# XIAOCHIZI/spark-bam

Measured on AMD Instinct MI355X. Metric: decompressed GB/s + records/sec (inflate+boundary check) at 1/2/4/8 MI355X, higher is better.
Workload: dtype u8

## Files before the change

### spark-bam_amd/csrc/inflate.hip

```cpp
#include "sbh_internal.h"

namespace sbh {
namespace {

#ifndef SBH_HUFF_WAVES
#define SBH_HUFF_WAVES 4
#endif
constexpr int LIT_FAST = 10;
constexpr int DIST_FAST = 8;
constexpr int CL_FAST = 7;
constexpr int PDIST_FAST = 10;
constexpr int WAVES = SBH_HUFF_WAVES;
#ifndef SBH_LZ_THREADS
#define SBH_LZ_THREADS 512
#endif
constexpr uint32_t LZ_THREADS = SBH_LZ_THREADS;
#ifndef SBH_LZ_SHORT
#define SBH_LZ_SHORT 32
#endif
constexpr uint32_t LZ_SHORT = SBH_LZ_SHORT;
static_assert(LZ_SHORT <= 33, "k_lz finds a short match's start within 32 slots back");
constexpr uint32_t TOK_PAIR = 1u << 24;
constexpr uint32_t TOK_MATCH = 0x80000000u;

// ... 1136 lines not shown

#ifndef SBH_ASM_REDO
#define SBH_ASM_REDO 1
#endif
__device__ __forceinline__ LaneRun redo_asm(const WaveSmem &t, const uint32_t *stage, uint32_t A, uint32_t stop,
                                            uint32_t limit, const Ckpt &ck, const LaneRun &sp) {
  const uint32_t stop2 = stop < limit ? stop : limit;
  if (A >= stop2) return LaneRun{A >= limit ? LR_PAST : LR_RUN, A, 0, 0};
  const uint32_t tabb = uni((uint32_t)reinterpret_cast<uintptr_t>(t.tab));
  const uint32_t stb = uni((uint32_t)reinterpret_cast<uintptr_t>(stage) + 8u);
  const uint32_t pkb = uni((uint32_t)reinterpret_cast<uintptr_t>(&t.pk[0][11]));
  const uint32_t sentb = uni((uint32_t)reinterpret_cast<uintptr_t>(t.sent));
  const uint32_t sentd = sentb + 288u * 4u;
  uint32_t pos = A, lo = stage[A >> 5], hi = stage[(A >> 5) + 1];
  uint32_t vt = 0, tselb = tabb, ntok = 0, acc = 0;
  const uint32_t bad_e = 1u | PE_SPECIAL;
  const uint32_t k1 = ck.p1, k2 = ck.p2, k3 = ck.p3;
  uint32_t e = 0, bits, a, nx, x, ex, val, np, tmp, r15, q, p11, p12, p13, p14, p15, d, sh;
  uint64_t sA, sB, sC, sD, sE, sv;
  asm volatile(
      "s_mov_b64 %[sv], exec\n"
      "L_top%=:\n\t"
      "v_alignbit_b32 %[bits], %[hi], %[lo], %[pos]\n\t"
      "v_and_b32 %[a], 0x3ff, %[bits]\n\t"
      "v_lshl_add_u32 %[a], %[a], 2, %[tselb]\n\t"
      "ds_read_b32 %[e], %[a]\n\t"
      "v_lshrrev_b32 %[a], 5, %[pos]\n\t"
      "v_lshl_add_u32 %[a], %[a], 2, %[stb]\n\t"
      "ds_read_b32 %[nx], %[a]\n\t"
      "v_cmp_eq_u32 %[sA], 0, %[vt]\n\t"
      "v_cmp_ge_u32 %[sC], %[pos], %[stop]\n\t"
      "v_cmp_eq_u32 %[sB], %[pos], %[k1]\n\t"
      "v_cmp_eq_u32 %[sE], %[pos], %[k2]\n\t"
      "s_or_b64 %[sC], %[sC], %[sB]\n\t"
      "v_cmp_eq_u32 %[sB], %[pos], %[k3]\n\t"
      "s_or_b64 %[sC], %[sC], %[sE]\n\t"
      "s_or_b64 %[sC], %[sC], %[sB]\n\t"
      "s_and_b64 %[sC], %[sC], %[sA]\n"
      "L_nock%=:\n\t"
      "s_waitcnt lgkmcnt(1)\n\t"
      "v_cmp_gt_i32 %[sD], 0, %[e]\n\t"
      "s_and_b64 %[sD], %[sD], exec\n\t"
      "s_cbranch_scc0 L_nosp%=\n\t"
      "v_and_b32 %[tmp], 0x4000, %[e]\n\t"
      "v_cmp_ne_u32 %[sB], 0, %[tmp]\n\t"
      "s_and_b64 %[sB], %[sB], %[sD]\n\t"
      "s_cbranch_scc0 L_nosp%=\n\t"
      "s_and_saveexec_b64 %[sB], %[sB]\n\t"
      "v_bfrev_b32 %[r15], %[bits]\n\t"
      "v_lshrrev_b32 %[r15], 17, %[r15]\n\t"
      "v_lshrrev_b32 %[q], 6, %[vt]\n\t"
      "v_add_u32 %[q], %[pkb], %[q]\n\t"
      "ds_read_b32 %[p11], %[q]\n\t"
      "ds_read_b32 %[p12], %[q] offset:4\n\t"
      "ds_read_b32 %[p13], %[q] offset:8\n\t"
      "ds_read_b32 %[p14], %[q] offset:12\n\t"
      "ds_read_b32 %[p15], %[q] offset:16\n\t"
      "s_waitcnt lgkmcnt(0)\n\t"
      "v_mov_b32 %[d], %[p11]\n\t"
      "v_mov_b32 %[sh], 4\n\t"
      "v_lshrrev_b32 %[tmp], 16, %[p11]\n\t"
      "v_cmp_le_u32 vcc, %[tmp], %[r15]\n\t"
      "s_nop 1\n\t"
      "v_cndmask_b32_e32 %[d], %[d], %[p12], vcc\n\t"
      "v_cndmask_b32_e64 %[sh], %[sh], 3, vcc\n\t"
      "v_lshrrev_b32 %[tmp], 16, %[p12]\n\t"
      "v_cmp_le_u32 vcc, %[tmp], %[r15]\n\t"
      "s_nop 1\n\t"
      "v_cndmask_b32_e32 %[d], %[d], %[p13], vcc\n\t"
      "v_cndmask_b32_e64 %[sh], %[sh], 2, vcc\n\t"
      "v_lshrrev_b32 %[tmp], 16, %[p13]\n\t"
      "v_cmp_le_u32 vcc, %[tmp], %[r15]\n\t"
      "s_nop 1\n\t"
      "v_cndmask_b32_e32 %[d], %[d], %[p14], vcc\n\t"
      "v_cndmask_b32_e64 %[sh], %[sh], 1, vcc\n\t"
      "v_lshrrev_b32 %[tmp], 16, %[p14]\n\t"
      "v_cmp_le_u32 vcc, %[tmp], %[r15]\n\t"
      "s_nop 1\n\t"
      "v_cndmask_b32_e32 %[d], %[d], %[p15], vcc\n\t"
      "v_cndmask_b32_e64 %[sh], %[sh], 0, vcc\n\t"
      "v_lshrrev_b32 %[tmp], %[sh], %[r15]\n\t"
      "v_add_u32 %[tmp], %[tmp], %[d]\n\t"
      "v_and_b32 %[tmp], 0xffff, %[tmp]\n\t"
      "v_min_u32 %[tmp], 0x13f, %[tmp]\n\t"
      "v_cmp_ne_u32 vcc, 0, %[vt]\n\t"
      "v_mov_b32 %[q], %[sentd]\n\t"
      "v_mov_b32 %[d], %[sentb]\n\t"
      "v_cndmask_b32_e32 %[q], %[d], %[q], vcc\n\t"
      "v_lshl_add_u32 %[tmp], %[tmp], 2, %[q]\n\t"
      "ds_read_b32 %[e], %[tmp]\n\t"
      "v_lshrrev_b32 %[tmp], 16, %[p15]\n\t"
      "v_cmp_ge_u32 vcc, %[r15], %[tmp]\n\t"
      "s_waitcnt lgkmcnt(0)\n\t"
      "s_nop 1\n\t"
      "v_cndmask_b32_e32 %[e], %[e], %[bad_e], vcc\n\t"
      "s_mov_b64 exec, %[sB]\n\t"
      "v_cmp_gt_i32 %[sD], 0, %[e]\n"
      "L_nosp%=:\n\t"
      "s_or_b64 %[sD], %[sD], %[sC]\n\t"
      "s_andn2_b64 exec, exec, %[sD]\n\t"
      "s_cbranch_execz L_end%=\n\t"
      "v_and_b32 %[tmp], 31, %[e]\n\t"
      "v_bfe_u32 %[x], %[e], 5, 4\n\t"
      "v_bfe_u32 %[ex], %[bits], %[e], %[x]\n\t"
      "v_add3_u32 %[np], %[pos], %[tmp], %[x]\n\t"
      "v_add_u32_sdwa %[val], %[ex], %[e] dst_sel:DWORD dst_unused:UNUSED_PAD src0_sel:DWORD src1_sel:WORD_1\n\t"
      "v_xor_b32 %[tmp], %[np], %[pos]\n\t"
      "v_cmp_lt_u32 vcc, 31, %[tmp]\n\t"
      "v_and_b32 %[vt], 0x1000, %[e]\n\t"
      "v_mov_b32 %[pos], %[np]\n\t"
      "s_waitcnt lgkmcnt(0)\n\t"
      "v_cndmask_b32_e32 %[lo], %[lo], %[hi], vcc\n\t"
      "v_cndmask_b32_e32 %[hi], %[hi], %[nx], vcc\n\t"
      "v_addc_co_u32_e64 %[ntok], vcc, 0, %[ntok], %[sA]\n\t"
      "v_add_u32 %[tselb], %[tabb], %[vt]\n\t"
      "v_mad_u32_u24 %[acc], %[vt], %[val], %[acc]\n\t"
      "v_and_b32 %[tmp], 0x400, %[e]\n\t"
      "v_lshl_add_u32 %[acc], %[tmp], 2, %[acc]\n\t"
      "s_branch L_top%=\n"
      "L_end%=:\n\t"
      "s_waitcnt lgkmcnt(0)\n\t"
      "s_mov_b64 exec, %[sv]"
      : [pos] "+v"(pos), [lo] "+v"(lo), [hi] "+v"(hi), [vt] "+v"(vt), [tselb] "+v"(tselb), [ntok] "+v"(ntok),
        [acc] "+v"(acc), [e] "+v"(e), [bits] "=&v"(bits), [a] "=&v"(a), [nx] "=&v"(nx), [x] "=&v"(x),
        [ex] "=&v"(ex), [val] "=&v"(val), [np] "=&v"(np), [tmp] "=&v"(tmp), [r15] "=&v"(r15), [q] "=&v"(q),
        [p11] "=&v"(p11), [p12] "=&v"(p12), [p13] "=&v"(p13), [p14] "=&v"(p14), [p15] "=&v"(p15), [d] "=&v"(d),
        [sh] "=&v"(sh), [sA] "=&s"(sA), [sB] "=&s"(sB), [sC] "=&s"(sC), [sD] "=&s"(sD), [sE] "=&s"(sE),
        [sv] "=&s"(sv)
      : [stop] "v"(stop2), [k1] "v"(k1), [k2] "v"(k2), [k3] "v"(k3), [tabb] "s"(tabb), [stb] "s"(stb),
        [pkb] "s"(pkb), [sentb] "s"(sentb), [sentd] "s"(sentd), [bad_e] "v"(bad_e)
      : "vcc", "scc", "memory");
  LaneRun r{LR_RUN, pos, ntok, ntok + (acc >> 12)};
  if (vt == 0 && (pos >= stop2 || pos == k1 || pos == k2 || pos == k3)) {
    if (pos < stop2) {
      const bool one = pos == k1;
      const bool two = pos == k2;
      r.ntok += sp.ntok - (one ? CK1 : two ? CK2 : CK3);
      r.nout += sp.nout - ck_out(ck, one, two);
      r.st = sp.st;
      r.exit = sp.exit;
    } else if (pos >= limit) {
      r.st = LR_PAST;
    }
  } else {
    r.st = (vt == 0 && (e & PE_EOB)) ? LR_EOB : LR_DEAD;
    r.exit = pos + (e & 31);
  }
  return r;
}

#ifndef SBH_ASM_EMIT
#define SBH_ASM_EMIT 1
#endif
__device__ __forceinline__ void emit_asm(const WaveSmem &t, const uint32_t *stage, uint32_t A, uint32_t stop,
                                         uint32_t limit, uint32_t *tk, uint32_t tidx, uint32_t out0, uint32_t &bad) {
  const uint32_t stop2 = stop < limit ? stop : limit;
  if (A >= stop2) return;
  const uint32_t tabb = uni((uint32_t)reinterpret_cast<uintptr_t>(t.tab));
  const uint32_t stb = uni((uint32_t)reinterpret_cast<uintptr_t>(stage) + 8u);
  const uint32_t pkb = uni((uint32_t)reinterpret_cast<uintptr_t>(&t.pk[0][11]));
  const uint32_t sentb = uni((uint32_t)reinterpret_cast<uintptr_t>(t.sent));
  const uint32_t sentd = sentb + 288u * 4u;
  const uint64_t tkp = reinterpret_cast<uint64_t>(tk);
  const uint64_t tkb = (uint64_t)uni((uint32_t)tkp) | (uint64_t)uni((uint32_t)(tkp >> 32)) << 32;
  uint32_t pos = A, lo = stage[A >> 5], hi = stage[(A >> 5) + 1];
  uint32_t vt = 0, tselb = tabb, ntok = 0, acc = 0, ml = 0, voff = tidx * 4u, badv = 0, cnt = 0;
  const uint32_t om1 = out0 - 1u;
  const uint32_t bad_e = 1u | PE_SPECIAL;
  uint32_t e = 0, bits, a, nx, x, ex, val, np, tmp, r15, q, p11, p12, p13, p14, p15, d, sh, vtok, vb;
  uint64_t sA, sB, sC, sD, sE, sL, sBad, sv;
  asm volatile(
      "s_mov_b64 %[sv], exec\n\t"
      "s_mov_b64 %[sBad], 0\n"
      "L_top%=:\n\t"
      "v_alignbit_b32 %[bits], %[hi], %[lo], %[pos]\n\t"
      "v_and_b32 %[a], 0x3ff, %[bits]\n\t"
      "v_lshl_add_u32 %[a], %[a], 2, %[tselb]\n\t"
      "ds_read_b32 %[e], %[a]\n\t"
      "v_lshrrev_b32 %[a], 5, %[pos]\n\t"
      "v_lshl_add_u32 %[a], %[a], 2, %[stb]\n\t"
      "ds_read_b32 %[nx], %[a]\n\t"
      "v_cmp_eq_u32 %[sA], 0, %[vt]\n\t"
      "v_cmp_ge_u32 %[sC], %[pos], %[stop]\n\t"
      "s_and_b64 %[sC], %[sC], %[sA]\n"
      "L_nock%=:\n\t"
      "s_waitcnt lgkmcnt(1)\n\t"
      "v_cmp_gt_i32 %[sD], 0, %[e]\n\t"
      "s_and_b64 %[sD], %[sD], exec\n\t"
      "s_cbranch_scc0 L_nosp%=\n\t"
      "v_and_b32 %[tmp], 0x4000, %[e]\n\t"
      "v_cmp_ne_u32 %[sB], 0, %[tmp]\n\t"
      "s_and_b64 %[sB], %[sB], %[sD]\n\t"
      "s_cbranch_scc0 L_nosp%=\n\t"
      "s_and_saveexec_b64 %[sB], %[sB]\n\t"
      "v_bfrev_b32 %[r15], %[bits]\n\t"
      "v_lshrrev_b32 %[r15], 17, %[r15]\n\t"
      "v_lshrrev_b32 %[q], 6, %[vt]\n\t"
      "v_add_u32 %[q], %[pkb], %[q]\n\t"
      "ds_read_b32 %[p11], %[q]\n\t"
      "ds_read_b32 %[p12], %[q] offset:4\n\t"
      "ds_read_b32 %[p13], %[q] offset:8\n\t"
      "ds_read_b32 %[p14], %[q] offset:12\n\t"
      "ds_read_b32 %[p15], %[q] offset:16\n\t"
      "s_waitcnt lgkmcnt(0)\n\t"
      "v_mov_b32 %[d], %[p11]\n\t"
      "v_mov_b32 %[sh], 4\n\t"
      "v_lshrrev_b32 %[tmp], 16, %[p11]\n\t"
      "v_cmp_le_u32 vcc, %[tmp], %[r15]\n\t"
      "s_nop 1\n\t"
      "v_cndmask_b32_e32 %[d], %[d], %[p12], vcc\n\t"
      "v_cndmask_b32_e64 %[sh], %[sh], 3, vcc\n\t"
      "v_lshrrev_b32 %[tmp], 16, %[p12]\n\t"
      "v_cmp_le_u32 vcc, %[tmp], %[r15]\n\t"
      "s_nop 1\n\t"
      "v_cndmask_b32_e32 %[d], %[d], %[p13], vcc\n\t"
      "v_cndmask_b32_e64 %[sh], %[sh], 2, vcc\n\t"
      "v_lshrrev_b32 %[tmp], 16, %[p13]\n\t"
      "v_cmp_le_u32 vcc, %[tmp], %[r15]\n\t"
      "s_nop 1\n\t"
      "v_cndmask_b32_e32 %[d], %[d], %[p14], vcc\n\t"
      "v_cndmask_b32_e64 %[sh], %[sh], 1, vcc\n\t"
      "v_lshrrev_b32 %[tmp], 16, %[p14]\n\t"
      "v_cmp_le_u32 vcc, %[tmp], %[r15]\n\t"
      "s_nop 1\n\t"
      "v_cndmask_b32_e32 %[d], %[d], %[p15], vcc\n\t"
      "v_cndmask_b32_e64 %[sh], %[sh], 0, vcc\n\t"
      "v_lshrrev_b32 %[tmp], %[sh], %[r15]\n\t"
      "v_add_u32 %[tmp], %[tmp], %[d]\n\t"
      "v_and_b32 %[tmp], 0xffff, %[tmp]\n\t"
      "v_min_u32 %[tmp], 0x13f, %[tmp]\n\t"
      "v_cmp_ne_u32 vcc, 0, %[vt]\n\t"
      "v_mov_b32 %[q], %[sentd]\n\t"
      "v_mov_b32 %[d], %[sentb]\n\t"
      "v_cndmask_b32_e32 %[q], %[d], %[q], vcc\n\t"
      "v_lshl_add_u32 %[tmp], %[tmp], 2, %[q]\n\t"
      "ds_read_b32 %[e], %[tmp]\n\t"
      "v_lshrrev_b32 %[tmp], 16, %[p15]\n\t"
      "v_cmp_ge_u32 vcc, %[r15], %[tmp]\n\t"
      "s_waitcnt lgkmcnt(0)\n\t"
      "s_nop 1\n\t"
      "v_cndmask_b32_e32 %[e], %[e], %[bad_e], vcc\n\t"
      "s_mov_b64 exec, %[sB]\n\t"
      "v_cmp_gt_i32 %[sD], 0, %[e]\n"
      "L_nosp%=:\n\t"
      "s_or_b64 %[sD], %[sD], %[sC]\n\t"
      "s_andn2_b64 exec, exec, %[sD]\n\t"
      "s_cbranch_execz L_end%=\n\t"
      "v_and_b32 %[tmp], 31, %[e]\n\t"
      "v_bfe_u32 %[x], %[e], 5, 4\n\t"
      "v_bfe_u32 %[ex], %[bits], %[e], %[x]\n\t"
      "v_add3_u32 %[np], %[pos], %[tmp], %[x]\n\t"
      "v_add_u32_sdwa %[val], %[ex], %[e] dst_sel:DWORD dst_unused:UNUSED_PAD src0_sel:DWORD src1_sel:WORD_1\n\t"
      "v_and_b32 %[vt], 0x1000, %[e]\n\t"
      "v_xor_b32 %[tmp], %[np], %[pos]\n\t"
      "v_cmp_ne_u32 %[sL], 0, %[vt]\n\t"
      "v_cmp_lt_u32 vcc, 31, %[tmp]\n\t"
      "v_mov_b32 %[pos], %[np]\n\t"
      "v_lshlrev_b32 %[vtok], 8, %[val]\n\t"
      "v_and_b32 %[tmp], 0x600, %[e]\n\t"
      "v_lshl_or_b32 %[vtok], %[tmp], 14, %[vtok]\n\t"
      "v_or_b32 %[np], %[ml], %[val]\n\t"
      "v_lshl_add_u32 %[ml], %[val], 16, %[mlk]\n\t"
      "v_cndmask_b32_e64 %[vtok], %[np], %[vtok], %[sA]\n\t"
      "s_waitcnt lgkmcnt(0)\n\t"
      "v_cndmask_b32_e32 %[lo], %[lo], %[hi], vcc\n\t"
      "v_cndmask_b32_e32 %[hi], %[hi], %[nx], vcc\n\t"
      "s_and_b64 %[sE], %[sA], %[sL]\n\t"
      "s_mov_b64 %[sB], exec\n\t"
      "s_andn2_b64 exec, exec, %[sE]\n\t"
      "v_mov_b32 v124, v125\n\t"
      "v_mov_b32 v125, v126\n\t"
      "v_mov_b32 v126, v127\n\t"
      "v_mov_b32 v127, %[vtok]\n\t"
      "v_add_u32 %[cnt], 1, %[cnt]\n\t"
      "v_cmp_eq_u32 %[sE], 4, %[cnt]\n\t"
      "s_and_b64 exec, exec, %[sE]\n\t"
      "s_cbranch_execz L_nofl%=\n\t"
      "global_store_dwordx4 %[voff], v[124:127], %[tkb]\n\t"
      "s_nop 1\n\t"
      "v_add_u32 %[voff], 16, %[voff]\n\t"
      "v_mov_b32 %[cnt], 0\n"
      "L_nofl%=:\n\t"
      "s_mov_b64 exec, %[sB]\n\t"
      "v_add_u32 %[tselb], %[tabb], %[vt]\n\t"
      "s_branch L_top%=\n"
      "L_end%=:\n\t"
      "s_waitcnt lgkmcnt(0)\n\t"
      "s_mov_b64 exec, %[sv]\n\t"
      "v_cmp_le_u32 %[sE], 1, %[cnt]\n\t"
      "s_and_b64 exec, exec, %[sE]\n\t"
      "s_cbranch_execz L_fld%=\n\t"
      "v_lshl_add_u32 %[tmp], %[cnt], 2, %[voff]\n\t"
      "global_store_dword %[tmp], v127, %[tkb] offset:-4\n\t"
      "v_cmp_le_u32 %[sE], 2, %[cnt]\n\t"
      "s_and_b64 exec, exec, %[sE]\n\t"
      "global_store_dword %[tmp], v126, %[tkb] offset:-8\n\t"
      "v_cmp_le_u32 %[sE], 3, %[cnt]\n\t"
      "s_and_b64 exec, exec, %[sE]\n\t"
      "global_store_dword %[tmp], v125, %[tkb] offset:-12\n"
      "L_fld%=:\n\t"
      "s_mov_b64 exec, %[sv]\n\t"
      "v_cndmask_b32_e64 %[badv], 0, 1, %[sBad]"
      : [pos] "+v"(pos), [lo] "+v"(lo), [hi] "+v"(hi), [vt] "+v"(vt), [tselb] "+v"(tselb), [ntok] "+v"(ntok),
        [acc] "+v"(acc), [ml] "+v"(ml), [voff] "+v"(voff), [badv] "+v"(badv), [cnt] "+v"(cnt), [e] "+v"(e),
        [bits] "=&v"(bits),
        [a] "=&v"(a), [nx] "=&v"(nx), [x] "=&v"(x), [ex] "=&v"(ex), [val] "=&v"(val), [np] "=&v"(np),
        [tmp] "=&v"(tmp), [r15] "=&v"(r15), [q] "=&v"(q), [p11] "=&v"(p11), [p12] "=&v"(p12), [p13] "=&v"(p13),
        [p14] "=&v"(p14), [p15] "=&v"(p15), [d] "=&v"(d), [sh] "=&v"(sh), [vtok] "=&v"(vtok),
        [vb] "=&v"(vb), [sA] "=&s"(sA), [sB] "=&s"(sB), [sC] "=&s"(sC), [sD] "=&s"(sD), [sE] "=&s"(sE),
        [sL] "=&s"(sL), [sBad] "=&s"(sBad), [sv] "=&s"(sv)
      : [stop] "v"(stop2), [tabb] "s"(tabb), [stb] "s"(stb), [pkb] "s"(pkb), [sentb] "s"(sentb),
        [sentd] "s"(sentd), [bad_e] "v"(bad_e), [om1] "v"(om1), [tkb] "s"(tkb), [mlk] "s"(0x80010000u)
      : "vcc", "scc", "memory"
      , "v124", "v125", "v126", "v127"
  );
  bad |= badv;
}

template <class SM, class S>
__device__ __forceinline__ bool hdr_walk(SM &t, const S &src, uint32_t p, uint32_t limit, uint32_t nlen,
                                         uint32_t ndist, uint32_t ncode, uint32_t lane, uint32_t &q_out,
                                         uint64_t *h1, uint64_t *h2) {
  if (lane < 19) t.cl_lens[CL_ORDER[lane]] = lane < ncode ? (uint8_t)(src.bits32(p + 17 + 3 * lane) & 7) : 0;
  __builtin_amdgcn_wave_barrier();
  bool ok = uni(build_table(t, t.cl_lens, 19, 2, t.lit, CL_FAST, lane)) == 0;
  if (h1) *h1 = __builtin_readcyclecounter();
  for (uint32_t w = lane; w < 320 / 4; w += WAVE) reinterpret_cast<uint32_t *>(t.lens)[w] = 0;
  __builtin_amdgcn_wave_barrier();
  const uint32_t total = nlen + ndist;
  uint32_t i = 0, prev = 0, q = p + 17 + 3 * ncode;
  const uint64_t below = (1ull << lane) - 1;
  while (ok && i < total && q <= limit) {
    const uint32_t b = src.bits32(q + lane);
    const uint32_t e = t.lit[b & ((1u << CL_FAST) - 1)];
    const uint32_t L = e & 31, sym = (e >> 8) & 31;
    const uint32_t xb = sym < 16 ? 0 : sym == 16 ? 2 : sym == 17 ? 3 : 7;
    const uint32_t xv = __builtin_amdgcn_ubfe(b, L, xb);
    const uint32_t rep = sym < 16 ? 1 : sym == 16 ? 3 + xv : sym == 17 ? 3 + xv : 11 + xv;
    const uint32_t pack = (L + xb) | (rep << 8);
    uint64_t M = 0;
    const uint32_t i0 = i, tot8 = uni(total << 8);
    uint32_t oi = uni(i0 << 8), inf, tw;
    asm volatile(
        "s_nop 3\n"
        "L_walk%=:\n\t"
        "v_readlane_b32 %[inf], %[pack], %[oi]\n\t"
        "s_bitset1_b64 %[M], %[oi]\n\t"
        "s_add_u32 %[oi], %[oi], %[inf]\n\t"
        "s_and_b32 %[tw], %[oi], 0xc0\n\t"
        "s_cbranch_scc1 L_wend%=\n\t"
        "s_cmp_lt_u32 %[oi], %[tot8]\n\t"
        "s_cbranch_scc1 L_walk%=\n"
        "L_wend%=:"
        : [M] "+s"(M), [oi] "+s"(oi), [inf] "=&s"(inf), [tw] "=&s"(tw)
        : [pack] "v"(pack), [tot8] "s"(tot8)
        : "scc");
    const uint32_t o = oi & 0xffu;
    i = oi >> 8;
    const bool mine = (M >> lane) & 1;
    uint32_t ex;
    {
      const uint32_t x = wave_incl_scan(mine ? rep : 0);
      ex = x - (mine ? rep : 0);
    }
    const uint32_t start = i0 + ex;
    const uint64_t N = M & __ballot(sym != 16);
    const uint64_t lowN = N & below;
    const uint32_t own = sym < 16 ? sym : 0;
    const uint32_t src_lane = lowN ? 63 - (uint32_t)__builtin_clzll(lowN) : 0;
    const uint32_t from = __shfl(own, src_lane, WAVE);
    const uint32_t val = sym == 16 ? (lowN ? from : prev) : own;
    if (M & 1 && __builtin_amdgcn_readfirstlane(sym) == 16 && i0 == 0) ok = false;
    if (mine && val != 0) {
      const uint32_t e = min(start + rep, total);
      const uint32_t v4 = val * 0x01010101u;
      for (uint32_t j = start; j < e;) {
        const uint32_t d = j < nlen ? j : 288 + j - nlen;
        const uint32_t seg_end = j < nlen ? min(e, nlen) : e;
        if ((d & 3) == 0 && j + 4 <= seg_end) {
          *reinterpret_cast<uint32_t *>(&t.lens[d]) = v4;
          j += 4;
        } else {
          t.lens[d] = (uint8_t)val;
          ++j;
        }
      }
    }
    const uint32_t top = 63 - (uint32_t)__builtin_clzll(M);
    prev = __builtin_amdgcn_readlane(val, top);
    q += o;
  }
  if (i != total || q > limit) ok = false;
  __builtin_amdgcn_wave_barrier();
  if (h2) *h2 = __builtin_readcyclecounter();
  if (ok && uni(t.lens[256]) == 0) ok = false;
  q_out = q;
  return ok;
}

template <uint32_t NT>
__device__ __forceinline__ void fill_ptables(WaveSmem &t, uint32_t tid) {
  uint32_t lj0[16], lj1[16];
#pragma unroll
  for (uint32_t v = 1; v <= 15; ++v) {
    lj0[v] = t.pk[0][v] >> 16;
    lj1[v] = t.pk[1][v] >> 16;
  }
#pragma unroll 4
  for (uint32_t i = tid; i < (1u << LIT_FAST); i += NT) t.lit[i] = ptable_lit_entry(t, lj0, i);
#pragma unroll 4
  for (uint32_t i = tid; i < (1u << PDIST_FAST); i += NT) t.dist[i] = ptable_entry(t, lj1, 1, PDIST_FAST, i);
}

template <class SM, class S>
__device__ __forceinline__ bool par_header(SM &sm, S src, uint32_t p, uint32_t limit, bool &fixed_built,
                                           uint32_t wid, uint32_t lane, uint32_t &psym, uint32_t &last) {
  constexpr uint32_t NT = SM::NT;
  WaveSmem &t = sm.t;
  auto fill_tables = [&]() { fill_ptables<NT>(t, wid * WAVE + lane); };
  const uint32_t hb = uni(src.bits32(p));
  last = hb & 1;
  const uint32_t type = (hb >> 1) & 3;
  if (p + 3 > limit || type == 0 || type == 3) return false;
  if (type == 1) {
    psym = p + 3;
    if (!fixed_built) {
      if (wid == 0) {
        for (uint32_t s = lane; s < 288; s += WAVE) t.lens[s] = s < 144 ? 8 : s < 256 ? 9 : s < 280 ? 7 : 8;
        __builtin_amdgcn_wave_barrier();
        ptable_meta(t, t.lens, 288, 0, lane);
      }
      if (wid == (NT > WAVE ? 1u : 0u)) {
        if (lane < 32) t.lens[288 + lane] = 5;
        __builtin_amdgcn_wave_barrier();
        ptable_meta(t, t.lens + 288, 32, 1, lane);
      }
      __syncthreads();
      fill_tables();
      __syncthreads();
      fixed_built = true;
    }
    return true;
  }
  fixed_built = false;
  const uint32_t nlen = ((hb >> 3) & 31) + 257, ndist = ((hb >> 8) & 31) + 1, ncode = ((hb >> 13) & 15) + 4;
  if (nlen > 286 || ndist > 30) return false;
#ifdef SBH_HUFF_PROBE
  const uint64_t h0 = __builtin_readcyclecounter();
  uint64_t h1 = 0, h2 = 0;
#endif
  if (wid == 0) {
    uint32_t q;
#ifdef SBH_HUFF_PROBE
    const bool ok = hdr_walk(t, src, p, limit, nlen, ndist, ncode, lane, q, &h1, &h2);
#else
    const bool ok = hdr_walk(t, src, p, limit, nlen, ndist, ncode, lane, q, nullptr, nullptr);
#endif
    if (lane == 0) {
      sm.ctl[5] = ok;
      sm.ctl[6] = q;
    }
  }
  __syncthreads();
  if (!uni(sm.ctl[5])) return false;
  psym = uni(sm.ctl[6]);
  bool bad = false;
  if (wid == 0) bad = ptable_meta(t, t.lens, nlen, 0, lane) == 1;
  if (wid == (NT > WAVE ? 1u : 0u)) bad = bad || ptable_meta(t, t.lens + 288, ndist, 1, lane) == 1;
  if (__syncthreads_or(bad)) return false;
  fill_tables();
  __syncthreads();
#ifdef SBH_HUFF_PROBE
  if (NT == HT && wid == 0 && lane == 0) {
    atomicAdd(&hp_acc[8], h1 - h0);
    atomicAdd(&hp_acc[9], h2 - h1);
    atomicAdd(&hp_acc[10], __builtin_readcyclecounter() - h2);
  }
#endif
  return true;
}

constexpr uint32_t PAR_OK = 0, PAR_FAIL = 1, PAR_TAIL = 2;
template <bool LDS, class SM>
__device__ __forceinline__ uint32_t inflate_par(SM &sm, const uint8_t *__restrict__ dbase, uint32_t skip,
                            uint32_t limit, uint32_t usize, uint32_t *__restrict__ tk, uint32_t tid, uint32_t lane,
                            uint32_t wid, uint32_t &ntok_out, bool pre, uint32_t pre_psym, uint32_t pre_last,
                            uint32_t out_before, bool tail_ok, uint32_t *tail_p, uint32_t *tail_out) {
  constexpr uint32_t NT = SM::NT;
  const Src<LDS, SM::SDW> src{LDS ? sm.stage : reinterpret_cast<const uint32_t *>(dbase)};
  uint32_t p = skip, out = 0, ntok = 0;
  bool fixed_built = false;
  for (;;) {
#ifdef SBH_HUFF_PROBE
    const uint64_t tp0 = __builtin_readcyclecounter();
#endif
    uint32_t p0, last;
    if (pre) {
      p0 = pre_psym;
      last = pre_last;
      pre = false;
    } else if (!par_header(sm, src, p, limit, fixed_built, wid, lane, p0, last)) {
      return PAR_FAIL;
    }

#ifdef SBH_HUFF_PROBE
    const uint64_t tph = __builtin_readcyclecounter();
#endif
    uint32_t S = (limit > p0 ? limit - p0 : 0) / NT + 1;
    if (S < MIN_SLICE) S = MIN_SLICE;
    const uint32_t s = p0 + tid * S, stop = s + S;
    uint32_t A = s, nobad = 0;
    Ckpt ck;
    const LaneRun none{};
#if SBH_ASM_SPEC
    LaneRun r = LDS ? spec_asm(sm.t, sm.stage, A, stop, limit, ck)
                    : lane_run<RUN_SPEC>(sm.t, src, A, stop, limit, ck, none, nullptr, 0, nobad);
#else
    LaneRun r = lane_run<RUN_SPEC>(sm.t, src, A, stop, limit, ck, none, nullptr, 0, nobad);
#endif
    const LaneRun r1 = r;
    uint32_t *xa = sm.exitv, *xb = sm.exitv2;
    xa[tid] = r.st == LR_RUN ? r.exit : NOPOS;
    __syncthreads();
#ifdef SBH_HUFF_PROBE
    uint32_t nrounds = 0;
    __syncthreads();
    const uint64_t tp1 = __builtin_readcyclecounter();
#endif
    for (;;) {
#ifdef SBH_HUFF_PROBE
      ++nrounds;
#endif
      const uint32_t nA = tid == 0 ? p0 : xa[tid - 1];
      const bool changed = nA != NOPOS && nA != A;
      if (changed) {
        A = nA;
#if SBH_ASM_REDO
        r = LDS ? redo_asm(sm.t, sm.stage, A, stop, limit, ck, r1)
                : lane_run<RUN_REDO>(sm.t, src, A, stop, limit, ck, r1, nullptr, 0, nobad);
#else
        r = lane_run<RUN_REDO>(sm.t, src, A, stop, limit, ck, r1, nullptr, 0, nobad);
#endif
      }
      xb[tid] = r.st == LR_RUN ? r.exit : NOPOS;
      const bool again = __syncthreads_or(changed);
      uint32_t *const xt = xa;
      xa = xb;
      xb = xt;
#ifdef SBH_HUFF_PROBE
      if (SM::NT == HT && tid == 0 && nrounds == 1) atomicAdd(&hp_acc[12], __builtin_readcyclecounter() - tp1);
      if (SM::NT == HT && tid == 0 && nrounds == 2) atomicAdd(&hp_acc[13], __builtin_readcyclecounter() - tp1);
#endif
      if (!again) break;
    }
    uint32_t k, tpre, opre, ttot, otot, eob_end;
    {
      const uint64_t em = __ballot(r.st != LR_RUN);
      const uint32_t wf = em ? uni((uint32_t)__builtin_ctzll(em)) : (uint32_t)WAVE;
      const uint32_t it = wave_incl_scan(r.ntok), io = wave_incl_scan(r.nout);
      if (lane == WAVE - 1) {
        sm.wsum[wid] = it;
        sm.wsum2[wid] = io;
      }

      if (lane == (wf < WAVE ? wf : 0u)) {
        sm.wk[wid] = wf < WAVE ? tid : NT;
        sm.wkt[wid] = it;
        sm.wko[wid] = io;
        sm.wke[wid] = (r.st == LR_EOB && r.exit <= limit) ? r.exit : NOPOS;
      }
      __syncthreads();
      uint32_t bt = 0, bo = 0, at = 0, ao = 0;
      k = NT;
      ttot = otot = 0;
      eob_end = NOPOS;
#pragma unroll
      for (uint32_t w = 0; w < NT / WAVE; ++w) {
        const uint32_t st = sm.wsum[w], so = sm.wsum2[w], wkw = sm.wk[w];
        if (k == NT) {
          if (wkw < NT) {
            k = wkw;
            ttot = at + sm.wkt[w];
            otot = ao + sm.wko[w];
            eob_end = sm.wke[w];
          } else {
            at += st;
            ao += so;
          }
        }
        if (w < wid) {
          bt += st;
          bo += so;
        }
      }
      k = uni(k);
      ttot = uni(ttot);
      otot = uni(otot);
      eob_end = uni(eob_end);
      tpre = bt + it - r.ntok;
      opre = bo + io - r.nout;
    }
#ifdef SBH_HUFF_PROBE
    const uint64_t tp3 = __builtin_readcyclecounter();
    if (SM::NT == HT && tid == 0) {
      atomicAdd(&hp_acc[1], tph - tp0);
      atomicAdd(&hp_acc[2], tp1 - tph);
      atomicAdd(&hp_acc[3], tp3 - tp1);
      atomicAdd(&hp_acc[5], (unsigned long long)nrounds);
      atomicAdd(&hp_acc[6], 1ull);
      atomicAdd(&hp_acc[11], (unsigned long long)ttot);
    }
#endif
    if (k >= NT || eob_end == NOPOS || otot > usize - out) return PAR_FAIL;
    uint32_t bad = 0;
    if (tid <= k) {
#if SBH_ASM_EMIT
      if (LDS)
        emit_asm(sm.t, sm.stage, A, stop, limit, tk + ntok, tpre, out_before + out + opre, bad);
      else
#endif
        lane_run<RUN_EMIT>(sm.t, src, A, stop, limit, ck, none, tk + ntok + tpre, out_before + out + opre, bad);
    }
    if (__syncthreads_or(bad)) return PAR_FAIL;
#ifdef SBH_HUFF_PROBE
    if (SM::NT == HT && tid == 0) atomicAdd(&hp_acc[4], __builtin_readcyclecounter() - tp3);
#endif
    ntok += ttot;
    out += otot;
    p = eob_end;
    if (last) break;
    if (tail_ok && (limit - p) * 4 < limit && ntok + 2 <= usize) {
      *tail_p = p;
      *tail_out = out;
      ntok_out = ntok;
      return PAR_TAIL;
    }
  }
  if (out != usize) return PAR_FAIL;
  ntok_out = ntok;
  return PAR_OK;
}

struct HdrSrc {
  const uint32_t *p;
  uint32_t n;
  __device__ __forceinline__ uint32_t bits32(uint32_t pos) const {
    const uint32_t i = pos >> 5;
    const uint32_t a = p[i < n ? i : n - 1], b = p[i + 1 < n ? i + 1 : n - 1];
    return __builtin_amdgcn_alignbit(b, a, pos & 31);
  }
};

struct HdrSmem {
  uint32_t lit[1 << CL_FAST];
  uint16_t sorted[320];
  uint8_t lens[320];
  uint8_t cl_lens[20];
  uint32_t cnt[2][16];
  uint32_t pk[2][16];
  uint32_t sent[320];
};

__device__ __forceinline__ bool huff_serial_block(const DevBlocks &bl, uint64_t b) {
  const uint32_t csize = bl.csize[b], hsize = bl.hsize[b], usize = bl.usize[b];
  return (bl.flags[b] & BLK_TRUNCATED) || usize > 65536u || usize < PAR_MIN_USIZE ||
         (int32_t)csize - (int32_t)hsize - 8 < 0;
}

#ifndef SBH_HDR_WAVES
#define SBH_HDR_WAVES 4
#endif
constexpr uint32_t HDR_WAVES = SBH_HDR_WAVES;

__device__ __forceinline__ bool tail_hdr_room(uint32_t n1, uint32_t usize) {
  return n1 <= usize && usize - n1 >= HDR_OUT_DW + 2;
}

template <bool TAIL>
__global__ __launch_bounds__(WAVE * HDR_WAVES) void k_hdr(const uint8_t *__restrict__ comp, DevBlocks bl,
                                                         uint64_t nblocks, uint32_t *__restrict__ tok) {
  __shared__ HdrSmem tw[HDR_WAVES];
  __shared__ uint32_t stagew[HDR_WAVES][HDR_STAGE_DW];
  const uint32_t lane = threadIdx.x & (WAVE - 1), wid = uni(threadIdx.x / WAVE);
  const uint64_t b = (uint64_t)blockIdx.x * HDR_WAVES + wid;
  if (b >= nblocks) return;
  if (TAIL ? uni(bl.status[b]) != INF_TAIL : huff_serial_block(bl, b)) return;
  HdrSmem &t = tw[wid];
  uint32_t *stage = stagew[wid];
  const uint64_t cstart = bl.cstart[b];
  const uint32_t csize = bl.csize[b], hsize = bl.hsize[b], usize = bl.usize[b];
  const uint32_t data_len = csize - hsize - 8;
  const uint64_t dbyte = cstart + hsize;
  uint32_t skip = (uint32_t)(dbyte & 3) * 8;
  uint32_t limit = skip + data_len * 8;
  const uint8_t *dbase = comp + (dbyte & ~3ull);
  if (TAIL) {
    const uint32_t n1 = uni(bl.ntok[b]);
    if (!tail_hdr_room(n1, usize)) return;
    const uint32_t p = uni(tok[bl.ustart[b] + n1]), pd = p >> 5;
    dbase += 4ull * pd;
    skip = p & 31;
    limit -= 32 * pd;
  }
  const uint32_t ndw = min((limit + 31) / 32 + 2, HDR_STAGE_DW);
  const uint32_t *g = reinterpret_cast<const uint32_t *>(dbase);
  {
    constexpr uint32_t R = (HDR_STAGE_DW + WAVE - 1) / WAVE;
    uint32_t v[R];
#pragma unroll
    for (uint32_t r = 0; r < R; ++r) v[r] = g[min(lane + r * WAVE, ndw - 1)];
#pragma unroll
    for (uint32_t r = 0; r < R; ++r)
      if (lane + r * WAVE < ndw) stage[lane + r * WAVE] = v[r];
  }
  __builtin_amdgcn_wave_barrier();
  uint32_t *out = tok + bl.ustart[b] + usize - HDR_OUT_DW;
  const HdrSrc src{stage, ndw};
  const uint32_t lim = min(limit, ndw * 32 > 96 ? ndw * 32 - 96 : 0u);
  const uint32_t hb = uni(src.bits32(skip));
  const uint32_t nlen = ((hb >> 3) & 31) + 257, ndist = ((hb >> 8) & 31) + 1, ncode = ((hb >> 13) & 15) + 4;
  bool ok = ((hb >> 1) & 3) == 2 && skip + 17 <= lim && nlen <= 286 && ndist <= 30;
  uint32_t q = 0;
  if (ok) ok = hdr_walk(t, src, skip, lim, nlen, ndist, ncode, lane, q, nullptr, nullptr);
  if (ok) {
    const uint32_t r0 = ptable_meta(t, t.lens, nlen, 0, lane);
    const uint32_t r1 = ptable_meta(t, t.lens + 288, ndist, 1, lane);
    ok = r0 != 1 && r1 != 1;
  }
  __builtin_amdgcn_wave_barrier();
  if (ok) {
    uint32_t lj0[16], lj1[16];
#pragma unroll
    for (uint32_t v = 1; v <= 15; ++v) {
      lj0[v] = t.pk[0][v] >> 16;
      lj1[v] = t.pk[1][v] >> 16;
    }
#pragma unroll 4
    for (uint32_t i = lane; i < (1u << LIT_FAST); i += WAVE) out[i] = ptable_lit_entry(t, lj0, i);
#pragma unroll 4
    for (uint32_t i = lane; i < (1u << PDIST_FAST); i += WAVE)
      out[(1u << LIT_FAST) + i] = ptable_entry(t, lj1, 1, PDIST_FAST, i);
    for (uint32_t i = lane; i < 320; i += WAVE) out[HDR_SENT + i] = t.sent[i];
    if (lane < 32) out[HDR_PK + lane] = t.pk[lane >> 4][lane & 15];
    if (lane == 0) {
      out[HDR_PSYM] = q;
      out[HDR_LAST] = hb & 1;
    }
  }
  if (lane == 0) out[HDR_STATUS] = ok ? HDR_OK : 0u;
}

#ifdef SBH_HUFF_PROBE
__device__ void huff_probe_done(uint32_t tid, uint64_t nblocks, uint64_t hk0, bool timed) {
  if (tid != 0) return;
  if (timed) {
    atomicAdd(&hp_acc[7], __builtin_readcyclecounter() - hk0);
    atomicAdd(&hp_acc[14], 1ull);
  }
  __threadfence();
  if (atomicAdd(&hp_done, 1u) == (uint32_t)nblocks - 1) {
    unsigned long long a[15];
    for (int k = 0; k < 15; ++k) a[k] = atomicExch(&hp_acc[k], 0ull);
    hp_done = 0;
    const double n = (double)(a[14] ? a[14] : 1), d = (double)(a[6] ? a[6] : 1);
    printf("huffprobe blocks %llu (parallel %.0f) deflate %.0f per-BGZF-block cycles: stage %.0f hdr %.0f (cl %.0f walk %.0f tables %.0f) p1 %.0f p2 %.0f (rounds/defl %.2f) p3 %.0f whole %.0f tokens/defl %.0f | p2 to end of round1 %.0f round2 %.0f\n",
           (unsigned long long)nblocks, n, d, a[0] / n, a[1] / n, a[8] / n, a[9] / n, a[10] / n, a[2] / n, a[3] / n,
           a[5] / d, a[4] / n, a[7] / n, a[11] / d, a[12] / n, a[13] / n);
  }
}
#endif

// ... 687 lines not shown
```

Baseline: 218.8.

## Unroll emit_asm decode loop by four tokens with explicit length/distance sub-steps

Restructures the hand-written emit assembly loop from a single per-symbol state machine (with a vt state toggle, a token counter and register shifting) into four unrolled token iterations. Each iteration decodes a literal/length symbol and, when it is a length, immediately decodes the distance symbol under a nested exec mask. Tokens go straight into v124..v127 and are flushed with one dwordx4 store, so the per-symbol register rotation, counter compare and state-select table address are gone. It also removes the never-set bad-flag output and unused registers. The cost is much larger code, more SGPR masks and more divergent branching inside each iteration, and partial tails are now handled through the sX exec masks.

```diff
diff --git a/spark-bam_amd/csrc/inflate.hip b/spark-bam_amd/csrc/inflate.hip
--- a/spark-bam_amd/csrc/inflate.hip
+++ b/spark-bam_amd/csrc/inflate.hip
@@ -1312,170 +1312,190 @@
 #ifndef SBH_ASM_EMIT
 #define SBH_ASM_EMIT 1
 #endif
+#define SBH_EMIT_SLOW(PK, SENT)                                                                        \
+      "s_and_saveexec_b64 %[sS], %[sS]\n\t"                                                            \
+      "v_bfrev_b32 %[r15], %[bits]\n\t"                                                                \
+      "v_lshrrev_b32 %[r15], 17, %[r15]\n\t"                                                           \
+      "v_mov_b32 %[q], " PK "\n\t"                                                                     \
+      "ds_read_b32 %[p11], %[q]\n\t"                                                                   \
+      "ds_read_b32 %[p12], %[q] offset:4\n\t"                                                          \
+      "ds_read_b32 %[p13], %[q] offset:8\n\t"                                                          \
+      "ds_read_b32 %[p14], %[q] offset:12\n\t"                                                         \
+      "ds_read_b32 %[p15], %[q] offset:16\n\t"                                                         \
+      "s_waitcnt lgkmcnt(0)\n\t"                                                                       \
+      "v_mov_b32 %[d], %[p11]\n\t"                                                                     \
+      "v_mov_b32 %[sh], 4\n\t"                                                                         \
+      "v_lshrrev_b32 %[tmp], 16, %[p11]\n\t"                                                           \
+      "v_cmp_le_u32 vcc, %[tmp], %[r15]\n\t"                                                           \
+      "s_nop 1\n\t"                                                                                    \
+      "v_cndmask_b32_e32 %[d], %[d], %[p12], vcc\n\t"                                                  \
+      "v_cndmask_b32_e64 %[sh], %[sh], 3, vcc\n\t"                                                     \
+      "v_lshrrev_b32 %[tmp], 16, %[p12]\n\t"                                                           \
+      "v_cmp_le_u32 vcc, %[tmp], %[r15]\n\t"                                                           \
+      "s_nop 1\n\t"                                                                                    \
+      "v_cndmask_b32_e32 %[d], %[d], %[p13], vcc\n\t"                                                  \
+      "v_cndmask_b32_e64 %[sh], %[sh], 2, vcc\n\t"                                                     \
+      "v_lshrrev_b32 %[tmp], 16, %[p13]\n\t"                                                           \
+      "v_cmp_le_u32 vcc, %[tmp], %[r15]\n\t"                                                           \
+      "s_nop 1\n\t"                                                                                    \
+      "v_cndmask_b32_e32 %[d], %[d], %[p14], vcc\n\t"                                                  \
+      "v_cndmask_b32_e64 %[sh], %[sh], 1, vcc\n\t"                                                     \
+      "v_lshrrev_b32 %[tmp], 16, %[p14]\n\t"                                                           \
+      "v_cmp_le_u32 vcc, %[tmp], %[r15]\n\t"                                                           \
+      "s_nop 1\n\t"                                                                                    \
+      "v_cndmask_b32_e32 %[d], %[d], %[p15], vcc\n\t"                                                  \
+      "v_cndmask_b32_e64 %[sh], %[sh], 0, vcc\n\t"                                                     \
+      "v_lshrrev_b32 %[tmp], %[sh], %[r15]\n\t"              \
+      "v_add_u32 %[tmp], %[tmp], %[d]\n\t"                                                             \
+      "v_and_b32 %[tmp], 0xffff, %[tmp]\n\t"                                                           \
+      "v_min_u32 %[tmp], 0x13f, %[tmp]\n\t"     \
+      "v_lshl_add_u32 %[tmp], %[tmp], 2, " SENT "\n\t"                                                 \
+      "ds_read_b32 %[e], %[tmp]\n\t"                                                                   \
+      "v_lshrrev_b32 %[tmp], 16, %[p15]\n\t"                                                           \
+      "v_cmp_ge_u32 vcc, %[r15], %[tmp]\n\t"                                                           \
+      "s_waitcnt lgkmcnt(0)\n\t"                                                                       \
+      "s_nop 1\n\t"                                                                                    \
+      "v_cndmask_b32_e32 %[e], %[e], %[bad_e], vcc\n\t"                                                \
+      "s_mov_b64 exec, %[sS]\n\t"                                                                      \
+      "v_cmp_gt_i32 %[sD], 0, %[e]\n\t"
+#define SBH_EMIT_LOOKUP(TAB)                                                                           \
+      "v_alignbit_b32 %[bits], %[hi], %[lo], %[pos]\n\t"                                               \
+      "v_and_b32 %[a], 0x3ff, %[bits]\n\t"                                                             \
+      "v_lshl_add_u32 %[a], %[a], 2, " TAB "\n\t"                                                      \
+      "ds_read_b32 %[e], %[a]\n\t"                                                                     \
+      "v_lshrrev_b32 %[a], 5, %[pos]\n\t"                                                              \
+      "v_lshl_add_u32 %[a], %[a], 2, %[stb]\n\t"                                                       \
+      "ds_read_b32 %[nx], %[a]\n\t"
+#define SBH_EMIT_VALUE                                                                                 \
+      "v_and_b32 %[tmp], 31, %[e]\n\t"                                                                 \
+      "v_bfe_u32 %[x], %[e], 5, 4\n\t"                                                                 \
+      "v_bfe_u32 %[ex], %[bits], %[e], %[x]\n\t"                                                       \
+      "v_add3_u32 %[np], %[pos], %[tmp], %[x]\n\t"                                                     \
+      "v_add_u32_sdwa %[val], %[ex], %[e] dst_sel:DWORD dst_unused:UNUSED_PAD src0_sel:DWORD src1_sel:WORD_1\n\t" \
+      "v_xor_b32 %[tmp], %[np], %[pos]\n\t"                                                            \
+      "v_cmp_lt_u32 vcc, 31, %[tmp]\n\t"                                                               \
+      "v_mov_b32 %[pos], %[np]\n\t"
+#define SBH_EMIT_WINDOW                                                                                \
+      "s_waitcnt lgkmcnt(0)\n\t"                                                                       \
+      "v_cndmask_b32_e32 %[lo], %[lo], %[hi], vcc\n\t"                                                 \
+      "v_cndmask_b32_e32 %[hi], %[hi], %[nx], vcc\n\t"
+#define SBH_EMIT_ITER(J, VT, XJ)                                                                       \
+      "L_it" J "_%=:\n\t"                                                                              \
+      SBH_EMIT_LOOKUP("%[tabb]")                                                                       \
+      "v_cmp_ge_u32 %[sC], %[pos], %[stop]\n\t"     \
+      "s_waitcnt lgkmcnt(1)\n\t"                                                                       \
+      "v_cmp_gt_i32 %[sD], 0, %[e]\n\t"                                           \
+      "s_and_b64 %[sD], %[sD], exec\n\t"                                                               \
+      "s_cbranch_scc0 L_nosp" J "_%=\n\t"                                                              \
+      "v_and_b32 %[tmp], 0x4000, %[e]\n\t"                                                \
+      "v_cmp_ne_u32 %[sS], 0, %[tmp]\n\t"                                                              \
+      "s_and_b64 %[sS], %[sS], %[sD]\n\t"                                                              \
+      "s_cbranch_scc0 L_nosp" J "_%=\n\t"                                                              \
+      SBH_EMIT_SLOW("%[pkl]", "%[sentb]")                                                              \
+      "\nL_nosp" J "_%=:\n\t"                                                                          \
+                                             \
+      "s_or_b64 %[sD], %[sD], %[sC]\n\t"                                                               \
+      XJ                                                                                               \
+      "s_andn2_b64 exec, exec, %[sD]\n\t"                                                              \
+      "s_cbranch_execz L_end%=\n\t"                                                                    \
+      SBH_EMIT_VALUE                                                                                   \
+      "v_and_b32 %[q], 0x1000, %[e]\n\t"                                                   \
+         \
+      "v_lshlrev_b32 " VT ", 8, %[val]\n\t"                                                            \
+      "v_cmp_ne_u32 %[sL], 0, %[q]\n\t"                                                                \
+      "v_and_b32 %[tmp], 0x600, %[e]\n\t"                                                              \
+      "v_lshl_or_b32 " VT ", %[tmp], 14, " VT "\n\t"                                                   \
+      SBH_EMIT_WINDOW                                                                                  \
+      "s_and_b64 %[sL], %[sL], exec\n\t"                                                               \
+      "s_cbranch_scc0 L_nolen" J "_%=\n\t"                                                             \
+                  \
+      "s_and_saveexec_b64 %[sM], %[sL]\n\t"                                                            \
+      "v_lshl_add_u32 %[ml], %[val], 16, %[mlk]\n\t"                     \
+      SBH_EMIT_LOOKUP("%[tabd]")                                                                       \
+      "s_waitcnt lgkmcnt(1)\n\t"                                                                       \
+      "v_cmp_gt_i32 %[sD], 0, %[e]\n\t"                                                                \
+      "s_and_b64 %[sD], %[sD], exec\n\t"                                                               \
+      "s_cbranch_scc0 L_dok" J "_%=\n\t"                                                               \
+      "v_and_b32 %[tmp], 0x4000, %[e]\n\t"                                                             \
+      "v_cmp_ne_u32 %[sS], 0, %[tmp]\n\t"                                                              \
+      "s_and_b64 %[sS], %[sS], %[sD]\n\t"                                                              \
+      "s_cbranch_scc0 L_dsp" J "_%=\n\t"                                                               \
+      SBH_EMIT_SLOW("%[pkd]", "%[sentd]")                                                              \
+      "s_and_b64 %[sD], %[sD], exec\n\t"                                                               \
+      "s_cbranch_scc0 L_dok" J "_%=\n"                                                                 \
+      "L_dsp" J "_%=:\n\t"  \
+      "s_waitcnt lgkmcnt(0)\n\t"                                                                       \
+      XJ                                                                                               \
+      "s_andn2_b64 %[sM], %[sM], %[sD]\n\t"                                                            \
+      "s_cbranch_scc0 L_end%=\n\t"                                                                     \
+      "s_andn2_b64 exec, exec, %[sD]\n\t"                                                              \
+      "s_cbranch_execz L_dend" J "_%=\n"                                                               \
+      "L_dok" J "_%=:\n\t"                                                                             \
+      SBH_EMIT_VALUE                                                                                   \
+      "v_or_b32 " VT ", %[ml], %[val]\n\t"                                                             \
+      SBH_EMIT_WINDOW                                                                                  \
+      "\nL_dend" J "_%=:\n\t"                                                                          \
+      "s_mov_b64 exec, %[sM]\n"                                                                        \
+      "L_nolen" J "_%=:\n\t"
 __device__ __forceinline__ void emit_asm(const WaveSmem &t, const uint32_t *stage, uint32_t A, uint32_t stop,
-                                         uint32_t limit, uint32_t *tk, uint32_t tidx, uint32_t out0, uint32_t &bad) {
+                                         uint32_t limit, uint32_t *tk, uint32_t tidx) {
   const uint32_t stop2 = stop < limit ? stop : limit;
   if (A >= stop2) return;
   const uint32_t tabb = uni((uint32_t)reinterpret_cast<uintptr_t>(t.tab));
+  const uint32_t tabd = tabb + PE_LEN;
   const uint32_t stb = uni((uint32_t)reinterpret_cast<uintptr_t>(stage) + 8u);
-  const uint32_t pkb = uni((uint32_t)reinterpret_cast<uintptr_t>(&t.pk[0][11]));
+  const uint32_t pkl = uni((uint32_t)reinterpret_cast<uintptr_t>(&t.pk[0][11]));
+  const uint32_t pkd = uni((uint32_t)reinterpret_cast<uintptr_t>(&t.pk[1][11]));
   const uint32_t sentb = uni((uint32_t)reinterpret_cast<uintptr_t>(t.sent));
   const uint32_t sentd = sentb + 288u * 4u;
   const uint64_t tkp = reinterpret_cast<uint64_t>(tk);
   const uint64_t tkb = (uint64_t)uni((uint32_t)tkp) | (uint64_t)uni((uint32_t)(tkp >> 32)) << 32;
   uint32_t pos = A, lo = stage[A >> 5], hi = stage[(A >> 5) + 1];
-  uint32_t vt = 0, tselb = tabb, ntok = 0, acc = 0, ml = 0, voff = tidx * 4u, badv = 0, cnt = 0;
-  const uint32_t om1 = out0 - 1u;
+  uint32_t voff = tidx * 4u;
   const uint32_t bad_e = 1u | PE_SPECIAL;
-  uint32_t e = 0, bits, a, nx, x, ex, val, np, tmp, r15, q, p11, p12, p13, p14, p15, d, sh, vtok, vb;
-  uint64_t sA, sB, sC, sD, sE, sL, sBad, sv;
+  uint32_t e, bits, a, nx, x, ex, val, np, tmp, r15, q, p11, p12, p13, p14, p15, d, sh, ml;
+  uint64_t sC, sD, sS, sL, sM, sX1, sX2, sX3, sv;
   asm volatile(
       "s_mov_b64 %[sv], exec\n\t"
-      "s_mov_b64 %[sBad], 0\n"
-      "L_top%=:\n\t"
-      "v_alignbit_b32 %[bits], %[hi], %[lo], %[pos]\n\t"
-      "v_and_b32 %[a], 0x3ff, %[bits]\n\t"
-      "v_lshl_add_u32 %[a], %[a], 2, %[tselb]\n\t"
-      "ds_read_b32 %[e], %[a]\n\t"
-      "v_lshrrev_b32 %[a], 5, %[pos]\n\t"
-      "v_lshl_add_u32 %[a], %[a], 2, %[stb]\n\t"
-      "ds_read_b32 %[nx], %[a]\n\t"
-      "v_cmp_eq_u32 %[sA], 0, %[vt]\n\t"
-      "v_cmp_ge_u32 %[sC], %[pos], %[stop]\n\t"
-      "s_and_b64 %[sC], %[sC], %[sA]\n"
-      "L_nock%=:\n\t"
-      "s_waitcnt lgkmcnt(1)\n\t"
-      "v_cmp_gt_i32 %[sD], 0, %[e]\n\t"
-      "s_and_b64 %[sD], %[sD], exec\n\t"
-      "s_cbranch_scc0 L_nosp%=\n\t"
-      "v_and_b32 %[tmp], 0x4000, %[e]\n\t"
-      "v_cmp_ne_u32 %[sB], 0, %[tmp]\n\t"
-      "s_and_b64 %[sB], %[sB], %[sD]\n\t"
-      "s_cbranch_scc0 L_nosp%=\n\t"
-      "s_and_saveexec_b64 %[sB], %[sB]\n\t"
-      "v_bfrev_b32 %[r15], %[bits]\n\t"
-      "v_lshrrev_b32 %[r15], 17, %[r15]\n\t"
-      "v_lshrrev_b32 %[q], 6, %[vt]\n\t"
-      "v_add_u32 %[q], %[pkb], %[q]\n\t"
-      "ds_read_b32 %[p11], %[q]\n\t"
-      "ds_read_b32 %[p12], %[q] offset:4\n\t"
-      "ds_read_b32 %[p13], %[q] offset:8\n\t"
-      "ds_read_b32 %[p14], %[q] offset:12\n\t"
-      "ds_read_b32 %[p15], %[q] offset:16\n\t"
-      "s_waitcnt lgkmcnt(0)\n\t"
-      "v_mov_b32 %[d], %[p11]\n\t"
-      "v_mov_b32 %[sh], 4\n\t"
-      "v_lshrrev_b32 %[tmp], 16, %[p11]\n\t"
-      "v_cmp_le_u32 vcc, %[tmp], %[r15]\n\t"
-      "s_nop 1\n\t"
-      "v_cndmask_b32_e32 %[d], %[d], %[p12], vcc\n\t"
-      "v_cndmask_b32_e64 %[sh], %[sh], 3, vcc\n\t"
-      "v_lshrrev_b32 %[tmp], 16, %[p12]\n\t"
-      "v_cmp_le_u32 vcc, %[tmp], %[r15]\n\t"
-      "s_nop 1\n\t"
-      "v_cndmask_b32_e32 %[d], %[d], %[p13], vcc\n\t"
-      "v_cndmask_b32_e64 %[sh], %[sh], 2, vcc\n\t"
-      "v_lshrrev_b32 %[tmp], 16, %[p13]\n\t"
-      "v_cmp_le_u32 vcc, %[tmp], %[r15]\n\t"
-      "s_nop 1\n\t"
-      "v_cndmask_b32_e32 %[d], %[d], %[p14], vcc\n\t"
-      "v_cndmask_b32_e64 %[sh], %[sh], 1, vcc\n\t"
-      "v_lshrrev_b32 %[tmp], 16, %[p14]\n\t"
-      "v_cmp_le_u32 vcc, %[tmp], %[r15]\n\t"
-      "s_nop 1\n\t"
-      "v_cndmask_b32_e32 %[d], %[d], %[p15], vcc\n\t"
-      "v_cndmask_b32_e64 %[sh], %[sh], 0, vcc\n\t"
-      "v_lshrrev_b32 %[tmp], %[sh], %[r15]\n\t"
-      "v_add_u32 %[tmp], %[tmp], %[d]\n\t"
-      "v_and_b32 %[tmp], 0xffff, %[tmp]\n\t"
-      "v_min_u32 %[tmp], 0x13f, %[tmp]\n\t"
-      "v_cmp_ne_u32 vcc, 0, %[vt]\n\t"
-      "v_mov_b32 %[q], %[sentd]\n\t"
-      "v_mov_b32 %[d], %[sentb]\n\t"
-      "v_cndmask_b32_e32 %[q], %[d], %[q], vcc\n\t"
-      "v_lshl_add_u32 %[tmp], %[tmp], 2, %[q]\n\t"
-      "ds_read_b32 %[e], %[tmp]\n\t"
-      "v_lshrrev_b32 %[tmp], 16, %[p15]\n\t"
-      "v_cmp_ge_u32 vcc, %[r15], %[tmp]\n\t"
-      "s_waitcnt lgkmcnt(0)\n\t"
-      "s_nop 1\n\t"
-      "v_cndmask_b32_e32 %[e], %[e], %[bad_e], vcc\n\t"
-      "s_mov_b64 exec, %[sB]\n\t"
-      "v_cmp_gt_i32 %[sD], 0, %[e]\n"
-      "L_nosp%=:\n\t"
-      "s_or_b64 %[sD], %[sD], %[sC]\n\t"
-      "s_andn2_b64 exec, exec, %[sD]\n\t"
-      "s_cbranch_execz L_end%=\n\t"
-      "v_and_b32 %[tmp], 31, %[e]\n\t"
-      "v_bfe_u32 %[x], %[e], 5, 4\n\t"
-      "v_bfe_u32 %[ex], %[bits], %[e], %[x]\n\t"
-      "v_add3_u32 %[np], %[pos], %[tmp], %[x]\n\t"
-      "v_add_u32_sdwa %[val], %[ex], %[e] dst_sel:DWORD dst_unused:UNUSED_PAD src0_sel:DWORD src1_sel:WORD_1\n\t"
-      "v_and_b32 %[vt], 0x1000, %[e]\n\t"
-      "v_xor_b32 %[tmp], %[np], %[pos]\n\t"
-      "v_cmp_ne_u32 %[sL], 0, %[vt]\n\t"
-      "v_cmp_lt_u32 vcc, 31, %[tmp]\n\t"
-      "v_mov_b32 %[pos], %[np]\n\t"
-      "v_lshlrev_b32 %[vtok], 8, %[val]\n\t"
-      "v_and_b32 %[tmp], 0x600, %[e]\n\t"
-      "v_lshl_or_b32 %[vtok], %[tmp], 14, %[vtok]\n\t"
-      "v_or_b32 %[np], %[ml], %[val]\n\t"
-      "v_lshl_add_u32 %[ml], %[val], 16, %[mlk]\n\t"
-      "v_cndmask_b32_e64 %[vtok], %[np], %[vtok], %[sA]\n\t"
-      "s_waitcnt lgkmcnt(0)\n\t"
-      "v_cndmask_b32_e32 %[lo], %[lo], %[hi], vcc\n\t"
-      "v_cndmask_b32_e32 %[hi], %[hi], %[nx], vcc\n\t"
-      "s_and_b64 %[sE], %[sA], %[sL]\n\t"
-      "s_mov_b64 %[sB], exec\n\t"
-      "s_andn2_b64 exec, exec, %[sE]\n\t"
-      "v_mov_b32 v124, v125\n\t"
-      "v_mov_b32 v125, v126\n\t"
-      "v_mov_b32 v126, v127\n\t"
-      "v_mov_b32 v127, %[vtok]\n\t"
-      "v_add_u32 %[cnt], 1, %[cnt]\n\t"
-      "v_cmp_eq_u32 %[sE], 4, %[cnt]\n\t"
-      "s_and_b64 exec, exec, %[sE]\n\t"
-      "s_cbranch_execz L_nofl%=\n\t"
+      "s_mov_b64 %[sX1], 0\n\t"
+      "s_mov_b64 %[sX2], 0\n\t"
+      "s_mov_b64 %[sX3], 0\n"
+      SBH_EMIT_ITER("0", "v124", "")
+      SBH_EMIT_ITER("1", "v125", "s_or_b64 %[sX1], %[sX1], %[sD]\n\t")
+      SBH_EMIT_ITER("2", "v126", "s_or_b64 %[sX2], %[sX2], %[sD]\n\t")
+      SBH_EMIT_ITER("3", "v127", "s_or_b64 %[sX3], %[sX3], %[sD]\n\t")
       "global_store_dwordx4 %[voff], v[124:127], %[tkb]\n\t"
       "s_nop 1\n\t"
       "v_add_u32 %[voff], 16, %[voff]\n\t"
-      "v_mov_b32 %[cnt], 0\n"
-      "L_nofl%=:\n\t"
-      "s_mov_b64 exec, %[sB]\n\t"
-      "v_add_u32 %[tselb], %[tabb], %[vt]\n\t"
-      "s_branch L_top%=\n"
+      "s_branch L_it0_%=\n"
       "L_end%=:\n\t"
       "s_waitcnt lgkmcnt(0)\n\t"
-      "s_mov_b64 exec, %[sv]\n\t"
-      "v_cmp_le_u32 %[sE], 1, %[cnt]\n\t"
-      "s_and_b64 exec, exec, %[sE]\n\t"
+      "s_or_b64 %[sX2], %[sX2], %[sX3]\n\t"
+      "s_or_b64 %[sX1], %[sX1], %[sX2]\n\t"
+      "s_mov_b64 exec, %[sX1]\n\t"
       "s_cbranch_execz L_fld%=\n\t"
-      "v_lshl_add_u32 %[tmp], %[cnt], 2, %[voff]\n\t"
-      "global_store_dword %[tmp], v127, %[tkb] offset:-4\n\t"
-      "v_cmp_le_u32 %[sE], 2, %[cnt]\n\t"
-      "s_and_b64 exec, exec, %[sE]\n\t"
-      "global_store_dword %[tmp], v126, %[tkb] offset:-8\n\t"
-      "v_cmp_le_u32 %[sE], 3, %[cnt]\n\t"
-      "s_and_b64 exec, exec, %[sE]\n\t"
-      "global_store_dword %[tmp], v125, %[tkb] offset:-12\n"
+      "global_store_dword %[voff], v124, %[tkb]\n\t"
+      "s_mov_b64 exec, %[sX2]\n\t"
+      "global_store_dword %[voff], v125, %[tkb] offset:4\n\t"
+      "s_mov_b64 exec, %[sX3]\n\t"
+      "global_store_dword %[voff], v126, %[tkb] offset:8\n"
       "L_fld%=:\n\t"
-      "s_mov_b64 exec, %[sv]\n\t"
-      "v_cndmask_b32_e64 %[badv], 0, 1, %[sBad]"
-      : [pos] "+v"(pos), [lo] "+v"(lo), [hi] "+v"(hi), [vt] "+v"(vt), [tselb] "+v"(tselb), [ntok] "+v"(ntok),
-        [acc] "+v"(acc), [ml] "+v"(ml), [voff] "+v"(voff), [badv] "+v"(badv), [cnt] "+v"(cnt), [e] "+v"(e),
-        [bits] "=&v"(bits),
+      "s_mov_b64 exec, %[sv]"
+      : [pos] "+v"(pos), [lo] "+v"(lo), [hi] "+v"(hi), [voff] "+v"(voff), [e] "=&v"(e), [bits] "=&v"(bits),
         [a] "=&v"(a), [nx] "=&v"(nx), [x] "=&v"(x), [ex] "=&v"(ex), [val] "=&v"(val), [np] "=&v"(np),
         [tmp] "=&v"(tmp), [r15] "=&v"(r15), [q] "=&v"(q), [p11] "=&v"(p11), [p12] "=&v"(p12), [p13] "=&v"(p13),
-        [p14] "=&v"(p14), [p15] "=&v"(p15), [d] "=&v"(d), [sh] "=&v"(sh), [vtok] "=&v"(vtok),
-        [vb] "=&v"(vb), [sA] "=&s"(sA), [sB] "=&s"(sB), [sC] "=&s"(sC), [sD] "=&s"(sD), [sE] "=&s"(sE),
-        [sL] "=&s"(sL), [sBad] "=&s"(sBad), [sv] "=&s"(sv)
-      : [stop] "v"(stop2), [tabb] "s"(tabb), [stb] "s"(stb), [pkb] "s"(pkb), [sentb] "s"(sentb),
-        [sentd] "s"(sentd), [bad_e] "v"(bad_e), [om1] "v"(om1), [tkb] "s"(tkb), [mlk] "s"(0x80010000u)
-      : "vcc", "scc", "memory"
-      , "v124", "v125", "v126", "v127"
-  );
-  bad |= badv;
-}
+        [p14] "=&v"(p14), [p15] "=&v"(p15), [d] "=&v"(d), [sh] "=&v"(sh), [ml] "=&v"(ml), [sC] "=&s"(sC),
+        [sD] "=&s"(sD), [sS] "=&s"(sS), [sL] "=&s"(sL), [sM] "=&s"(sM), [sX1] "=&s"(sX1), [sX2] "=&s"(sX2),
+        [sX3] "=&s"(sX3), [sv] "=&s"(sv)
+      : [stop] "v"(stop2), [tabb] "s"(tabb), [tabd] "s"(tabd), [stb] "s"(stb), [pkl] "s"(pkl), [pkd] "s"(pkd),
+        [sentb] "s"(sentb), [sentd] "s"(sentd), [bad_e] "v"(bad_e), [tkb] "s"(tkb), [mlk] "s"(0x80010000u)
+      : "vcc", "scc", "memory", "v124", "v125", "v126", "v127");
+}
+#undef SBH_EMIT_ITER
+#undef SBH_EMIT_WINDOW
+#undef SBH_EMIT_VALUE
+#undef SBH_EMIT_LOOKUP
+#undef SBH_EMIT_SLOW
 
 template <class SM, class S>
 __device__ __forceinline__ bool hdr_walk(SM &t, const S &src, uint32_t p, uint32_t limit, uint32_t nlen,
@@ -1776,7 +1796,7 @@
     if (tid <= k) {
 #if SBH_ASM_EMIT
       if (LDS)
-        emit_asm(sm.t, sm.stage, A, stop, limit, tk + ntok, tpre, out_before + out + opre, bad);
+        emit_asm(sm.t, sm.stage, A, stop, limit, tk + ntok, tpre);
       else
 #endif
         lane_run<RUN_EMIT>(sm.t, src, A, stop, limit, ck, none, tk + ntok + tpre, out_before + out + opre, bad);
```

New measurement: 222.4, median of 6. 1.02x the previous value.
